# CVlab315/Domain-Adaptative-Hand-Pose-Estimation

Hardware: AMD Instinct MI355X
Metric: images/sec (unique source+target images per A+B+C training iteration, 2*B*N/t_iter) (higher is better)
Workload: dtype bf16; 1 GPU; RHD->H3D domain-adaptation iteration (steps A+B+C), resnet50 + 3-deconv neck + main head + 3 adversarial multiscale-fusion heads, 256x256, batch 64 source + 64 target per GPU, random init, synthetic batches; arch=resnet50, image_size=256, per_gpu_batch=64, global_batch=64, parallelism=dp1, hip_graphs=True, gradient_exchange=none (one rank)

## Files before the change

domain-adaptative-hand-pose-estimation_amd/csrc/api.hip:

```cpp
#include "common.h"
#include <stdarg.h>
#include <mutex>
#include <string>
#include <vector>

static thread_local char g_err[512] = "";
void mi355_set_error(const char* fmt, ...) {
  va_list ap; va_start(ap, fmt); vsnprintf(g_err, sizeof(g_err), fmt, ap); va_end(ap);
}
extern "C" const char* mi355_last_error(void) { return g_err; }
extern "C" int mi355_version(void) { return 100; }

namespace {
struct ProfState {
  std::mutex mu; bool on = false; int level = 0;
  std::vector<hipEvent_t> ev;
  std::vector<double> lflops, lbytes;
  std::vector<int> lfam; std::vector<std::string> llabel;
  size_t used = 0; double flops = 0, bytes = 0; long launches = 0;
};
ProfState& P() { static ProfState s; return s; }
thread_local char g_tag[160] = "";
}
bool prof_on() { return P().on; }
void prof_set_tag(const char* fmt, ...) {
  if (!P().on) return;
  va_list ap; va_start(ap, fmt); vsnprintf(g_tag, sizeof(g_tag), fmt, ap); va_end(ap);
}
ProfScope::ProfScope(hipStream_t st, double flops, double bytes, int family, const char* label) : s(st), on(false), slot(-1) {
  ProfState& p = P();
  if (!p.on || (family != 0 && p.level < 2)) return;
  std::lock_guard<std::mutex> lk(p.mu);
  if (p.used + 2 > p.ev.size()) {
    for (int i = 0; i < 2; ++i) { hipEvent_t e; if (hipEventCreate(&e) != hipSuccess) return; p.ev.push_back(e); }
  }
  slot = (int)p.used; p.used += 2; on = true;
  if (family == 0) { p.flops += flops; p.bytes += bytes; p.launches += 1; }
  if (p.lflops.size() < p.used / 2) { p.lflops.resize(p.used / 2); p.lbytes.resize(p.used / 2); p.lfam.resize(p.used / 2); p.llabel.resize(p.used / 2); }
  p.lflops[slot / 2] = flops; p.lbytes[slot / 2] = bytes; p.lfam[slot / 2] = family;
  p.llabel[slot / 2] = label ? label : g_tag;
  if (!label) g_tag[0] = 0;
  (void)hipEventRecord(p.ev[slot], s);
}
ProfScope::~ProfScope() {
  if (!on) return;
  ProfState& p = P();
  std::lock_guard<std::mutex> lk(p.mu);
  (void)hipEventRecord(p.ev[slot + 1], s);
}
extern "C" int mi355_prof_enable(int on) { P().on = on != 0; P().level = on; return MI355_OK; }
extern "C" int mi355_prof_reset(void) {
  ProfState& p = P(); std::lock_guard<std::mutex> lk(p.mu);
  p.used = 0; p.flops = 0; p.bytes = 0; p.launches = 0; return MI355_OK;
}
extern "C" int mi355_prof_read(double* total_ms, long* launches, double* flops, double* bytes) {
  ProfState& p = P(); std::lock_guard<std::mutex> lk(p.mu);
  double ms = 0;
  for (size_t i = 0; i + 1 < p.used; i += 2) {
    if (p.lfam[i / 2] != 0) continue;
    if (hipEventSynchronize(p.ev[i + 1]) != hipSuccess) MI_FAIL(MI355_ELAUNCH, "prof: event sync failed");
// ... 69 lines not shown
```

domain-adaptative-hand-pose-estimation_amd/csrc/common.h:

```cpp
#pragma once
#include <hip/hip_runtime.h>
#include <stdint.h>
#include <stdio.h>
#include <string.h>
#include "../../include/mi355pose.h"

typedef __bf16 bf16_t;
typedef __attribute__((ext_vector_type(8))) short bf16x8_t;
typedef __attribute__((ext_vector_type(4))) short bf16x4_t;
typedef __attribute__((ext_vector_type(16))) float f32x16_t;
typedef __attribute__((ext_vector_type(4))) float f32x4_t;

#define WAVE 64

void mi355_set_error(const char* fmt, ...);
#define MI_FAIL(code, ...) do { mi355_set_error(__VA_ARGS__); return (code); } while (0)
#define MI_CHECK_LAUNCH(name) do { hipError_t e_ = hipGetLastError(); \
  if (e_ != hipSuccess) MI_FAIL(MI355_ELAUNCH, "%s: %s", (name), hipGetErrorString(e_)); } while (0)

static inline hipStream_t as_stream(void* s) { return (hipStream_t)s; }
static inline int cdiv(long a, long b) { return (int)((a + b - 1) / b); }

template <typename T> struct Elem;
template <> struct Elem<float> {
// ... 84 lines not shown
  v = wave_max(v);
  __syncthreads();
  if ((threadIdx.x & 63) == 0) red[threadIdx.x >> 6] = v;
  __syncthreads();
  float r = red[0];
#pragma unroll
  for (int i = 1; i < NW; ++i) r = fmaxf(r, red[i]);
  return r;
}

struct FastDiv {
  unsigned mul, shr, d;
};
static inline FastDiv make_fastdiv(unsigned d) {
  FastDiv f; f.d = d;
  if (d == 1) { f.mul = 0; f.shr = 0; return f; }
  unsigned l = 0; while ((1ull << l) < d) ++l;
  unsigned long long m = ((1ull << 32) * ((1ull << l) - d)) / d + 1;
  f.mul = (unsigned)m; f.shr = l; return f;
}
__device__ inline unsigned fd_div(unsigned n, const FastDiv& f) {
  if (f.d == 1) return n;
  unsigned t = __umulhi(n, f.mul);
  return (t + ((n - t) >> 1)) >> (f.shr - 1);
}

struct ProfScope {
  hipStream_t s; bool on; int slot;
  ProfScope(hipStream_t st, double flops, double bytes = 0.0, int family = 0, const char* label = nullptr);
  ~ProfScope();
};
bool prof_on();
void prof_set_tag(const char* fmt, ...);
```

domain-adaptative-hand-pose-estimation_amd/csrc/igemm.hip:

```cpp
#include "common.h"
#include <stdlib.h>

#include "igemm_common.h"

template <typename T> struct MmaTraits;
template <> struct MmaTraits<bf16_t> { static constexpr int BK = 64; static constexpr int CH = 8; };
template <> struct MmaTraits<float> { static constexpr int BK = 32; static constexpr int CH = 4; };

#define GATHER_STAGES 1
template <typename T, int BM, int BN, int STAGES = 1, bool KW3 = false>
struct GatherSmem {
  static constexpr int kARows = KW3 ? BM + 4 * (BM / 8) + 4 : BM;
  static constexpr int kStage = (kARows + BN) * 128;
  static constexpr int kOutStride = BN * (int)sizeof(T) + 16;
  static constexpr int kOut = BM * kOutStride;
  static constexpr int kBytes = (STAGES * kStage > kOut ? STAGES * kStage : kOut) + BM * 4;
};

template <typename T, int BM, int BN, bool SMALL_C, int WGM = 2, int WGN = 2, bool HM_OUT = false, bool DMA = false, int EPI = 0,
          bool KW3 = false, bool CAT = false, int KG = 1>
__global__ __launch_bounds__(64 * WGM * WGN * KG, (KW3 && BM == 256) ? 2 : 1) void gather_gemm_kernel(const GatherArgs p) {
  constexpr int CH = MmaTraits<T>::CH;
  constexpr int GTHR = 64 * WGM * WGN;
  constexpr int NTHR = GTHR * KG, RPP = GTHR / 8;
// ... 1290 lines not shown
}

static bool t256_fits(const GatherArgs& a, long Mtot, int mode, long tmin) {
  (void)Mtot;
  long t = 0;
  for (int i = 0; i < a.nphase; ++i) t += cdiv(a.ph[i].M, 256L) * (a.Nout / 256);
  if (mode < 2) return t >= tmin && t <= 256;
  const long rem = t % 256;
  return t >= tmin && t <= 1024 && (rem == 0 || rem >= tmin);
}
template <typename T>
static int dispatch_gather(GatherArgs& a, hipStream_t st) {
  constexpr int CH = MmaTraits<T>::CH;
  if (a.Ci % CH) MI_FAIL(MI355_EINVAL, "gather: Ci=%d not a multiple of %d", a.Ci, CH);
  a.cshift = ilog2_exact(a.Ci / CH);
  if (a.cshift < 0) MI_FAIL(MI355_EINVAL, "gather: Ci/%d must be a power of two (Ci=%d)", CH, a.Ci);
  if (a.Nout % CH) MI_FAIL(MI355_EINVAL, "gather: Nout=%d not a multiple of %d", a.Nout, CH);
  if (a.nphase < 1 || a.nphase > 4) MI_FAIL(MI355_EINVAL, "gather: nphase=%d", a.nphase);
  long Mtot = 0, ntaps_tot = 0; int kchunks = 0; double flops = 0.0;
  for (int i = 0; i < a.nphase; ++i) {
    Mtot += a.ph[i].M; ntaps_tot += a.ph[i].ntaps;
    if ((a.ph[i].ntaps << a.cshift) > kchunks) kchunks = a.ph[i].ntaps << a.cshift;
    flops += 2.0 * a.ph[i].M * (double)a.Nout * a.ph[i].ntaps * a.Ci;
  }
  {
    const long imgs = a.ph[0].M / ((long)a.ph[0].OHp * a.ph[0].OWp);
    a.a_bytes = (unsigned)(imgs * a.Hi * a.Wi * a.Ci * (long)sizeof(T));
    a.b_bytes = (unsigned)((long)a.Nout * a.ldb * (long)sizeof(T));
  }
  const bool small = (a.Ci / CH) < 8;
  const long kavg = (ntaps_tot << a.cshift) / a.nphase;
  (void)kchunks;
  if (a.A2) flops += 2.0 * Mtot * (double)a.Nout * a.c2;
  ProfScope ps(st, flops, (double)a.a_bytes + (double)a.b_bytes * ntaps_tot / (a.ldb / a.Ci) + (double)Mtot * a.Nout * sizeof(T) +
                              (a.A2 ? (double)a.a2_bytes + a.b2_bytes : 0.0));
  static const int force = getenv("MI355_TILE") ? atoi(getenv("MI355_TILE")) : -1;
  static const int dma_mode = getenv("MI355_DMA") ? atoi(getenv("MI355_DMA")) : 1;
  if (a.A2) {
    if (small || a.nphase != 1 || a.out_sx != 1 || a.out_sy != 1 || a.bnb_partial || a.residual || a.accumulate)
      MI_FAIL(MI355_EINVAL, "concat-K forward: plain single-phase forward conv with >= 8 input chunks only");
    if (a.c2 < CH || a.c2 % CH || a.c2 > MmaTraits<T>::BK) MI_FAIL(MI355_EINVAL, "concat-K forward: c2=%d must be a multiple of %d and <= %d", a.c2, CH, MmaTraits<T>::BK);
    const long t128 = cdiv(Mtot, 128L) * cdiv(a.Nout, 128);
    static const int cat_tile = getenv("MI355_CAT_TILE") ? atoi(getenv("MI355_CAT_TILE")) : 0;
    static const int t256d_cat = getenv("MI355_T256D") ? atoi(getenv("MI355_T256D")) : 2;
    static const long t256d_cmin = getenv("MI355_T256D_MIN") ? atol(getenv("MI355_T256D_MIN")) : 192;
    if (t256d_cat >= 2 && sizeof(T) == 2 && a.Nout % 256 == 0 && dma_mode == 1 && t256_fits(a, Mtot, t256d_cat, t256d_cmin)) {
      if constexpr (sizeof(T) == 2) launch_gather<T, 256, 256, false, 2, 4, false, true, false, true>(a, st);
    }
    else if (cat_tile == 1 && a.Nout > 64) launch_gather<T, 128, 128, false, 2, 2, false, false, false, true>(a, st);
    else if (cat_tile == 2 && a.Nout > 64) launch_gather<T, 128, 128, false, 2, 2, false, true, false, true>(a, st);
    else if (cat_tile == 3 && a.Nout > 64) launch_gather<T, 64, 128, false, 2, 2, false, false, false, true>(a, st);
    else if (a.Nout <= 64) launch_gather<T, 64, 64, false, 2, 2, false, false, false, true>(a, st);
    else if ((dma_mode == 2) || (dma_mode == 1 && ((t128 >= 512 && kavg >= 128) || (t128 >= 256 && kavg >= 256)))) launch_gather<T, 128, 128, false, 2, 2, false, true, false, true>(a, st);
    else if (t128 >= 512 && kavg <= 32 && sizeof(T) == 2) launch_gather<T, 64, 128, false, 2, 2, false, false, false, true>(a, st);
    else if (t128 >= 512) launch_gather<T, 128, 128, false, 2, 2, false, false, false, true>(a, st);
    else if (cdiv(Mtot, 64L) * cdiv(a.Nout, 128) >= 512) launch_gather<T, 64, 128, false, 2, 2, false, false, false, true>(a, st);
    else launch_gather<T, 64, 64, false, 2, 2, false, false, false, true>(a, st);
    MI_CHECK_LAUNCH("gather_gemm_cat");
    return MI355_OK;
  }
  if constexpr (sizeof(T) == 2) {
    if (pgemm_eligible(a, 2)) return dispatch_pgemm(a, st);
  }
  if (small) { launch_gather<T, 128, 64, true>(a, st); }
  else if (force == 0) launch_gather<T, 128, 128, false>(a, st);
  else if (force == 1) launch_gather<T, 64, 128, false>(a, st);
  else if (force == 2) launch_gather<T, 128, 64, false>(a, st);
  else if (force == 3) launch_gather<T, 64, 64, false>(a, st);
  else {
    const long t128 = cdiv(Mtot, 128L) * cdiv(a.Nout, 128);
// ... 740 lines not shown
```

domain-adaptative-hand-pose-estimation_amd/csrc/igemm_common.h:

```cpp
#pragma once
#include "common.h"

#define MAX_TAPS 52
struct Tap { int8_t dy, dx; int16_t widx; };

struct Phase { int OHp, OWp, out_oy, out_ox, M, ntaps, tap0, ntm; };
struct GatherArgs {
  const void* A; const void* B; void* D;
  const float* bias; const void* residual; const float* scale;
  int Hi, Wi, Ci;
  int in_sy, in_sx;
  int Ho, Wo;
  int out_sy, out_sx;
  int Nout, ldb, ldd;
  int cshift;
  int accumulate;
  int nphase, ntn, ntiles;
  int hw;
  int lw;
  unsigned a_bytes, b_bytes;
  size_t stat_bytes;
  int stat_slices;
  const void* bnb_x; const void* bnb_y;
  const float* bnb_mean; const float* bnb_invstd; const float* bnb_gamma; const float* bnb_beta;
// ... 21 lines not shown
#pragma unroll
    for (int i = 0; i < 4; ++i)
      w[i] &= ((0u - ((mb >> (2 * i)) & 1u)) & 0x0000ffffu) | ((0u - ((mb >> (2 * i + 1)) & 1u)) & 0xffff0000u);
  } else {
#pragma unroll
    for (int i = 0; i < 4; ++i) w[i] &= 0u - ((mb >> i) & 1u);
  }
  return make_uint4(w[0], w[1], w[2], w[3]);
}

__device__ __forceinline__ int swz128(int r, int c) { return r * 128 + ((c ^ ((r >> 1) & 7)) << 4); }

__device__ __forceinline__ int xcd_remap(int bid, int nblk) {
  int q = nblk >> 3, r = nblk & 7, x = bid & 7, i = bid >> 3;
  int start = (x < r) ? x * (q + 1) : r * (q + 1) + (x - r) * q;
  return start + i;
}

typedef __attribute__((ext_vector_type(4))) unsigned int u32x4_t;
#define OOB_OFF ((int)0x80000000)
__device__ __forceinline__ __amdgpu_buffer_rsrc_t make_rsrc(const void* p, unsigned bytes) {
  return __builtin_amdgcn_make_buffer_rsrc(const_cast<void*>(p), 0, bytes, 0x00020000);
}
__device__ __forceinline__ uint4 buf_load16(__amdgpu_buffer_rsrc_t rs, int byte_off) {
  u32x4_t v = __builtin_amdgcn_raw_buffer_load_b128(rs, byte_off, 0, 0);
  return make_uint4(v[0], v[1], v[2], v[3]);
}
__device__ __forceinline__ unsigned buf_load4(__amdgpu_buffer_rsrc_t rs, int byte_off) {
  return __builtin_amdgcn_raw_buffer_load_b32(rs, byte_off, 0, 0);
}


bool pgemm_eligible(const GatherArgs& a, int elem_size);
int dispatch_pgemm(GatherArgs& a, hipStream_t st);

int dispatch_gather_fp8(GatherArgs& a, hipStream_t st);

void launch_slab_reduce(const float* ws, float* dw, long n, int S, long stride, int accumulate, hipStream_t st);
```

domain-adaptative-hand-pose-estimation_amd/csrc/pgemm.hip:

```cpp
#include "common.h"
#include <stdlib.h>

#include "igemm_common.h"

template <int BM, int BN, int NS>
struct PgSmem {
  static constexpr int kStage = BM * 128;
  static constexpr int kOut = BM * BN * 2;
  static constexpr int bytes(int nk) { return nk * BN * 128 + NS * kStage + kOut; }
};

template <int BN> __device__ __forceinline__ int out_swz(int r, int c) {
  if constexpr (BN == 128) return r * 256 + ((c ^ (r & 15)) << 4);
  else return r * 128 + ((c ^ ((r >> 1) & 7)) << 4);
}

typedef __attribute__((address_space(3))) char* lds_cptr;
__device__ __forceinline__ unsigned lds_addr(const void* p) { return (unsigned)(uintptr_t)(lds_cptr)(const_cast<void*>(p)); }
__device__ __forceinline__ bf16x8_t lds_read16(unsigned a) { bf16x8_t v; asm volatile("ds_read_b128 %0, %1" : "=v"(v) : "v"(a)); return v; }
__device__ __forceinline__ u32x4_t lds_read16u(unsigned a) { u32x4_t v; asm volatile("ds_read_b128 %0, %1" : "=v"(v) : "v"(a)); return v; }
__device__ __forceinline__ void lds_write8(unsigned a, uint2 v) { asm volatile("ds_write_b64 %0, %1" :: "v"(a), "v"(v) : "memory"); }
__device__ __forceinline__ void lds_write4(unsigned a, float v) { asm volatile("ds_write_b32 %0, %1" :: "v"(a), "v"(v) : "memory"); }
__device__ __forceinline__ float lds_read4(unsigned a) { float v; asm volatile("ds_read_b32 %0, %1" : "=v"(v) : "v"(a)); return v; }
#define LDS_WAIT_ALL() asm volatile("s_waitcnt lgkmcnt(0)" ::: "memory")
// ... 415 lines not shown
    asm volatile("s_waitcnt vmcnt(0)" ::: "memory");
    RAW_BARRIER();
    static_assert(NW * BN * 3 * 4 <= SM::kOut, "statistics scratch must fit in the staging region");
    if (lane < CPR) {
#pragma unroll
      for (int e = 0; e < CH; ++e) {
        const unsigned qa = out_base + (unsigned)(((wave * BN + ec * CH + e) * 3) * 4);
        lds_write4(qa, sn); lds_write4(qa + 4, smean[e]); lds_write4(qa + 8, sm2[e]);
      }
    }
    LDS_WAIT_ALL();
    RAW_BARRIER();
    if (t < BN && n0 + t < p.Nout) {
      float qn[NW], qm[NW], qv[NW];
#pragma unroll
      for (int w = 0; w < NW; ++w) {
        const unsigned qa = out_base + (unsigned)(((w * BN + t) * 3) * 4);
        qn[w] = lds_read4(qa); qm[w] = lds_read4(qa + 4); qv[w] = lds_read4(qa + 8);
      }
      asm volatile("s_waitcnt lgkmcnt(0)" : "+v"(qn[0]), "+v"(qn[1]), "+v"(qn[2]), "+v"(qn[3]), "+v"(qm[0]), "+v"(qm[1]), "+v"(qm[2]),
                   "+v"(qm[3]), "+v"(qv[0]), "+v"(qv[1]), "+v"(qv[2]), "+v"(qv[3]));
      float cn = 0.f, mean = 0.f, m2 = 0.f;
#pragma unroll
      for (int w = 0; w < NW; ++w) {
        const float nb = qn[w];
        if (nb > 0.f) { const float nt = cn + nb, f = nb / nt, d = qm[w] - mean; mean += d * f; m2 += qv[w] + d * d * cn * f; cn = nt; }
      }
      float* out = p.stat_partial + ((size_t)gm * p.Nout + n0 + t) * 3;
      out[0] = cn; out[1] = mean; out[2] = m2;
    }
  }
}

template <int BM, int BN, int NS, int EPI, bool ADD>
static void launch_pgemm_epi(GatherArgs& a, int ncu, int ntm, int smem, hipStream_t st) {
  auto kern = pgemm_kernel<BM, BN, NS, EPI, ADD>;
  static int attr = 0;
  if (smem > attr) { (void)hipFuncSetAttribute((const void*)kern, hipFuncAttributeMaxDynamicSharedMemorySize, smem); attr = smem; }
  static int occ_smem[4] = {0, 0, 0, 0}, occ_n[4] = {0, 0, 0, 0};
  int per_cu = 0;
  for (int i = 0; i < 4; ++i) if (occ_smem[i] == smem) per_cu = occ_n[i];
  if (!per_cu) {
    int nb = 0;
    if (hipOccupancyMaxActiveBlocksPerMultiprocessor(&nb, kern, 256, (size_t)smem) != hipSuccess || nb < 1) nb = 1;
    per_cu = nb;
    for (int i = 0; i < 4; ++i) if (!occ_smem[i]) { occ_smem[i] = smem; occ_n[i] = nb; break; }
  }
  static const int cap = getenv("MI355_PG_PER_CU") ? atoi(getenv("MI355_PG_PER_CU")) : 2;
  if (per_cu > cap) per_cu = cap;
  int groups = ncu * per_cu / a.ntn; if (groups < 1) groups = 1;
  if (groups > ntm) groups = ntm;
  if (EPI == 1) a.stat_slices = groups;
  hipLaunchKernelGGL(kern, dim3(groups * a.ntn), dim3(256), smem, st, a);
}
template <int BM, int BN, int NS>
static bool launch_pgemm(GatherArgs& a, int ncu, hipStream_t st) {
  const int nk = a.Ci >> 6;
  const bool add = a.residual || a.accumulate;
  a.pg_nadd = add ? (NS - 1) / nk + 2 : 0;
  const int smem = PgSmem<BM, BN, NS>::bytes(nk) + a.pg_nadd * (PgSmem<BM, BN, NS>::kOut + BM * BN / 8);
  if (smem > 160 * 1024) return false;
  const int ntm = cdiv(a.ph[0].M, BM);
  a.ntn = cdiv(a.Nout, BN);
  a.ph[0].ntm = ntm;
  a.ntiles = ntm * a.ntn;
  a.stat_slices = 0;
  if (a.stat_partial && (a.residual || a.accumulate || (size_t)ntm * a.Nout * 3 * sizeof(float) > a.stat_bytes)) a.stat_partial = nullptr;
  if (a.stat_partial) launch_pgemm_epi<BM, BN, NS, 1, false>(a, ncu, ntm, smem, st);
  else if (a.residual || a.accumulate) launch_pgemm_epi<BM, BN, NS, 0, true>(a, ncu, ntm, smem, st);
  else launch_pgemm_epi<BM, BN, NS, 0, false>(a, ncu, ntm, smem, st);
  return true;
}

static int g_pgemm_mode = -1;
extern "C" int mi355_set_pgemm(int mode) {
  const int prev = g_pgemm_mode;
  g_pgemm_mode = mode < 0 ? -1 : (mode > 2 ? 2 : mode);
  return prev;
}
static int pg_bn(const GatherArgs& a) {
  if (a.Nout > 64 && (long)a.Ci * 128 * 2 <= 64 * 1024) return 128;
  if ((long)a.Ci * 64 * 2 <= 64 * 1024) return 64;
  return 0;
}
bool pgemm_eligible(const GatherArgs& a, int elem_size) {
  static const int env_mode = getenv("MI355_PGEMM") ? atoi(getenv("MI355_PGEMM")) : 1;
  const int mode = g_pgemm_mode >= 0 ? g_pgemm_mode : env_mode;
  if (!mode || elem_size != 2) return false;
  if (a.nphase != 1 || a.ph[0].ntaps != 1 || a.A2) return false;
  const Tap& tp = a.taps[a.ph[0].tap0];
  if (tp.dy != 0 || tp.dx != 0 || tp.widx != 0) return false;
  if (a.in_sx != 1 || a.in_sy != 1 || a.out_sx != 1 || a.out_sy != 1) return false;
  if (a.ph[0].OHp != a.Hi || a.ph[0].OWp != a.Wi || a.Ho != a.Hi || a.Wo != a.Wi || a.ph[0].out_oy || a.ph[0].out_ox) return false;
  if (a.Ci % 64 || a.ldb != a.Ci || a.ldd != a.Nout || a.Nout % 8) return false;
  if (a.bnb_partial || a.hw) return false;
  const long Mrows = a.ph[0].M;
  if (Mrows * a.Ci * 2 >= (1L << 31) || Mrows * a.Nout * 2 >= (1L << 31)) return false;
  if (Mrows < 256 || !pg_bn(a)) return false;
  if (a.residual && a.accumulate) return false;
  if (a.acc_mask && (a.Nout % 32 || !a.accumulate)) return false;
  if (mode >= 2) return true;
  static const int add_maxk = getenv("MI355_PG_ADD") ? atoi(getenv("MI355_PG_ADD")) * 64 : 64;
  if ((a.residual || a.accumulate) && a.Ci > add_maxk) return false;
  static const long min_rows = getenv("MI355_PG_MIN_ROWS") ? atol(getenv("MI355_PG_MIN_ROWS")) : 32768;
  return Mrows >= min_rows && (a.Ci <= 128 || (a.Ci <= 256 && a.Nout <= 128));
}

int dispatch_pgemm(GatherArgs& a, hipStream_t st) {
  static int ncu = 0;
  if (!ncu) {
    int dev = 0, v = 0;
    if (hipGetDevice(&dev) != hipSuccess || hipDeviceGetAttribute(&v, hipDeviceAttributeMultiprocessorCount, dev) != hipSuccess || v < 1)
      MI_FAIL(MI355_ELAUNCH, "pgemm: cannot read the CU count");
    ncu = v;
  }
  static const int ring_env = getenv("MI355_PG_RING") ? atoi(getenv("MI355_PG_RING")) : 0;
  static const int bm = getenv("MI355_PG_BM") ? atoi(getenv("MI355_PG_BM")) : 64;
  const int bn = pg_bn(a);
  const int nk = a.Ci >> 6;
  int ring = ring_env;
  if (!ring) {
    const bool add = a.residual || a.accumulate;
    auto bytes = [&](int ns) { return nk * bn * 128 + ns * 64 * 128 + 64 * bn * 2 + (add ? ((ns - 1) / nk + 2) * (64 * bn * 2 + 64 * bn / 8) : 0); };
    if (!add) for (int ns : {8, 6, 5, 4}) if (!ring && bytes(ns) <= 80 * 1024) ring = ns;
    for (int ns : {8, 6, 5, 4}) if (!ring && bytes(ns) <= 160 * 1024) ring = ns;
    if (!ring) ring = 4;
  }
  bool ok = false;
  if (bn == 128) {
    if (bm == 128) ok = launch_pgemm<128, 128, 4>(a, ncu, st);
    else if (ring == 8) ok = launch_pgemm<64, 128, 8>(a, ncu, st);
    else if (ring == 6) ok = launch_pgemm<64, 128, 6>(a, ncu, st);
    else if (ring == 5) ok = launch_pgemm<64, 128, 5>(a, ncu, st);
    else ok = launch_pgemm<64, 128, 4>(a, ncu, st);
  } else {
    if (bm == 128) ok = launch_pgemm<128, 64, 4>(a, ncu, st);
    else if (ring == 8) ok = launch_pgemm<64, 64, 8>(a, ncu, st);
    else if (ring == 6) ok = launch_pgemm<64, 64, 6>(a, ncu, st);
    else if (ring == 5) ok = launch_pgemm<64, 64, 5>(a, ncu, st);
    else ok = launch_pgemm<64, 64, 4>(a, ncu, st);
  }
  if (!ok) MI_FAIL(MI355_EINVAL, "pgemm: the weight slice of K = %d channels does not fit LDS (bn %d)", a.Ci, bn);
  MI_CHECK_LAUNCH("pgemm");
  return MI355_OK;
}
```

profiles/insitu_table.py:

```python
import csv
import json
import re
import sys
import collections

trace, logf, iters = sys.argv[1], sys.argv[2], int(sys.argv[3])
MFMA, HBM = 1.75e15, 6.3e12

PAT = [('fwd8', 'gather_fp8_kernel'), ('dgrad8', 'gather_fp8_kernel'), ('fwd', ('gather_gemm_kernel', 'pgemm_kernel')),
       ('dgrad', ('gather_gemm_kernel', 'pgemm_kernel')), ('hm1x1', 'gather_gemm_kernel'), ('wgrad_kw_group', 'wgrad_kw_group_kernel'),
       ('wgrad_kw2', 'wgrad_kw2_kernel'), ('wgrad_kw', 'wgrad_kw_kernel'), ('wgrad_group256', 'wgrad_group256_kernel'), ('wgrad_group', 'wgrad_group_kernel'),
       ('wgrad8', 'wgrad_kw'), ('wgrad', 'wgrad_gemm_kernel'),
       ('bn_stats', 'bn_stats_kernel'), ('bn_finalize', 'bn_finalize'), ('bn_apply', 'bn_apply_kernel'), ('bn_relu_maxpool', 'bn_relu_maxpool_kernel'),
       ('bn_bwd_res', 'bn_bwd_resident_kernel'), ('bn_bwd_reduce', 'bn_bwd_reduce_kernel'), ('bn_bwd_finalize', 'bn_bwd_finalize_kernel'),
       ('bn_bwd_apply', 'bn_bwd_apply_kernel'), ('slab_reduce_group', 'slab_reduce_group_kernel'), ('slab_reduce', 'slab_reduce_kernel')]
FAMILY_KERNELS = {0: ('gather_gemm_kernel', 'gather_fp8_kernel', 'pgemm_kernel', 'wgrad_gemm_kernel', 'wgrad_kw_kernel', 'wgrad_kw2_kernel',
                      'wgrad_group_kernel', 'wgrad_group256_kernel', 'wgrad_kw_group_kernel', 'wgrad_kw8_kernel', 'wgrad_kw28_kernel'),
                  1: ('bn_stats_kernel', 'bn_finalize_kernel', 'bn_finalize_wide_kernel', 'bn_apply_kernel', 'bn_relu_maxpool_kernel',
                      'bn_bwd_resident_kernel', 'bn_bwd_reduce_kernel', 'bn_bwd_finalize_kernel', 'bn_bwd_apply_kernel'),
                  2: ('slab_reduce_kernel', 'slab_reduce_group_kernel')}


def base(name):
    m = re.match(r'_Z\d+([A-Za-z0-9_]+?)I', name)
    if m:
        return m.group(1)
    return re.sub(r'<.*|\(.*', '', re.sub(r'^void ', '', name)).strip()


log = json.load(open(logf))['launches']
rows = []
for r in csv.DictReader(open(trace)):
    rows.append((int(r['Start_Timestamp']), base(r['Kernel_Name']), r['Kernel_Name'], (int(r['End_Timestamp']) - int(r['Start_Timestamp'])) / 1e3,
                 int(r['Grid_Size_X']) // max(int(r['Workgroup_Size_X']), 1)))
rows.sort()
out = []
for fam in (0, 1, 2):
    ents = [e for e in log if e['family'] == fam]
    if not ents:
        continue
    ks = [r for r in rows if r[1] in FAMILY_KERNELS[fam]]
    if fam == 1:
        ks = [r for r in ks if not (r[1] == 'bn_bwd_reduce_kernel' and 'Lb0ELi0E' in r[2])]
    n = len(ents)
    if len(ks) < n * iters:
        print('# family %d: trace holds %d launches, fewer than %d x %d -- skipped' % (fam, len(ks), iters, n)); continue
    ks = ks[-n * iters:]
    bad = 0
    for j, e in enumerate(ents):
# ... 34 lines not shown
```

profiles/pgemm_bench.py:

```python
import os
import sys

import torch

ROOT = os.path.dirname(os.path.dirname(os.path.abspath(__file__)))
sys.path[:0] = [ROOT, os.path.join(ROOT, 'domain-adaptative-hand-pose-estimation_amd')]
import mi355
from mi355 import ops

dev = torch.device('cuda:0')
mi355.load()
dt = torch.bfloat16
LAYERS = [(64, 64, 64, 256, 8, 8), (64, 16, 256, 1024, 12, 12), (64, 32, 128, 512, 8, 8), (64, 16, 1024, 256, 10, 10),
          (64, 64, 256, 256, 3, 2), (64, 32, 512, 128, 6, 6), (64, 64, 256, 64, 4, 4), (64, 8, 512, 2048, 6, 6),
          (64, 8, 2048, 512, 4, 4), (64, 64, 256, 128, 2, 2), (64, 32, 256, 256, 3, 3), (64, 32, 512, 256, 2, 2),
          (64, 16, 1024, 512, 2, 2), (64, 64, 64, 64, 2, 2), (64, 16, 256, 256, 3, 2)]


def timeit(fn, n=20):
    for _ in range(2):
        fn()
    torch.cuda.synchronize()
    g = torch.cuda.CUDAGraph()
    st = torch.cuda.Stream()
# ... 23 lines not shown
        wf, wt = ops.pack_weights(wm, Co, 1, Ci, Ci, dt)
        x = ops.nhwc_empty(N, Ci, H, H, dt, dev).normal_()
        dy = ops.nhwc_empty(N, Co, H, H, dt, dev).normal_()
        cold = os.environ.get('COLD', '0') == '1'
        nrot = max(2, int(600e6 // (2 * N * H * H * (Ci + Co)) + 1)) if cold else 1
        xs = [x] + [x.clone() for _ in range(nrot - 1)]
        dys = [dy] + [dy.clone() for _ in range(nrot - 1)]
        rot = [0]

        def nxt(lst):
            rot[0] += 1
            return lst[rot[0] % nrot]
        M = N * H * H
        fl = 2.0 * M * Ci * Co
        by = 2.0 * (M * Ci + M * Co + Ci * Co)
        wb = wm.reshape(Co, Ci).to(dt).float()
        y = ops.conv_fwd(desc, x, wf)
        ref = x.permute(0, 2, 3, 1).reshape(M, Ci).float() @ wb.t()
        e_f = float((y.permute(0, 2, 3, 1).reshape(M, Co).float() - ref).abs().max() / (ref.abs().max() + 1e-6))
        ys, part = ops.conv_fwd_stats(desc, x, wf, None)
        e_s = float((ys.float() - y.float()).abs().max())
        dx = ops.conv_dgrad(desc, dy, wt)
        refd = dy.permute(0, 2, 3, 1).reshape(M, Co).float() @ wb
        e_d = float((dx.permute(0, 2, 3, 1).reshape(M, Ci).float() - refd).abs().max() / (refd.abs().max() + 1e-6))
        t_f = timeit(lambda: ops.conv_fwd(desc, nxt(xs), wf))
        t_s = timeit(lambda: ops.conv_fwd_stats(desc, nxt(xs), wf, None))
        t_d = timeit(lambda: ops.conv_dgrad(desc, nxt(dys), wt))
        tot['fwd'] += t_f * nf; tot['fwd_stats'] += t_s * nf; tot['dgrad'] += t_d * nd
        print('%s %4d->%4d @%2d  fwd %6.1f us %5.0f TF/s %5.0f GB/s | +stats %6.1f us | dgrad %6.1f us %5.0f TF/s | err %.1e %.1e stats-vs-plain %.1e'
              % (tag, Ci, Co, H, t_f * 1e6, fl / t_f / 1e12, by / t_f / 1e9, t_s * 1e6, t_d * 1e6, fl / t_d / 1e12, e_f, e_d, e_s), flush=True)
    print('%s per iteration: fwd %.3f ms (with statistics %.3f ms), dgrad %.3f ms' % (tag, tot['fwd'] * 1e3, tot['fwd_stats'] * 1e3, tot['dgrad'] * 1e3))


if __name__ == '__main__':
    main()
```

Baseline: 4275 images/s.

## Add full-width 256-column pointwise GEMM kernel for large 256-channel 1x1 convs

Adds a persistent pointwise GEMM kernel for 1x1 convolutions with 256 input channels and up to 256 outputs. Each 512-thread block covers the full output width, keeps all weights in registers and streams activation rows through a deep LDS ring filled by buffer-to-LDS loads. Hand-written MFMA inline asm does the math, and the epilogue can fuse bias, scale, ReLU and BN statistics, plus an optional concatenated second input. By default it is only used for large M (at least 128K rows, or 64K with concat), replacing the gather GEMM on those layers so activations are read once instead of once per column tile. The cost is a heavy register footprint and a new hand-scheduled code path that may not beat the existing kernel on every shape.

```diff
diff --git a/domain-adaptative-hand-pose-estimation_amd/csrc/api.hip b/domain-adaptative-hand-pose-estimation_amd/csrc/api.hip
--- a/domain-adaptative-hand-pose-estimation_amd/csrc/api.hip
+++ b/domain-adaptative-hand-pose-estimation_amd/csrc/api.hip
@@ -1,5 +1,6 @@
 #include "common.h"
 #include <stdarg.h>
+#include <string.h>
 #include <mutex>
 #include <string>
 #include <vector>
@@ -26,6 +27,11 @@
 void prof_set_tag(const char* fmt, ...) {
   if (!P().on) return;
   va_list ap; va_start(ap, fmt); vsnprintf(g_tag, sizeof(g_tag), fmt, ap); va_end(ap);
+}
+void prof_tag_suffix(const char* suffix) {
+  if (!P().on) return;
+  const size_t n = strlen(g_tag);
+  snprintf(g_tag + n, sizeof(g_tag) - n, "%s", suffix);
 }
 ProfScope::ProfScope(hipStream_t st, double flops, double bytes, int family, const char* label) : s(st), on(false), slot(-1) {
   ProfState& p = P();
diff --git a/domain-adaptative-hand-pose-estimation_amd/csrc/common.h b/domain-adaptative-hand-pose-estimation_amd/csrc/common.h
--- a/domain-adaptative-hand-pose-estimation_amd/csrc/common.h
+++ b/domain-adaptative-hand-pose-estimation_amd/csrc/common.h
@@ -140,3 +140,4 @@
 };
 bool prof_on();
 void prof_set_tag(const char* fmt, ...);
+void prof_tag_suffix(const char* suffix);
diff --git a/domain-adaptative-hand-pose-estimation_amd/csrc/igemm.hip b/domain-adaptative-hand-pose-estimation_amd/csrc/igemm.hip
--- a/domain-adaptative-hand-pose-estimation_amd/csrc/igemm.hip
+++ b/domain-adaptative-hand-pose-estimation_amd/csrc/igemm.hip
@@ -1346,10 +1346,13 @@
   const long kavg = (ntaps_tot << a.cshift) / a.nphase;
   (void)kchunks;
   if (a.A2) flops += 2.0 * Mtot * (double)a.Nout * a.c2;
+  const bool wide = sizeof(T) == 2 && pgemm_wide_takes(a, 2);
+  if (wide && prof_on()) prof_tag_suffix(" pgw");
   ProfScope ps(st, flops, (double)a.a_bytes + (double)a.b_bytes * ntaps_tot / (a.ldb / a.Ci) + (double)Mtot * a.Nout * sizeof(T) +
                               (a.A2 ? (double)a.a2_bytes + a.b2_bytes : 0.0));
   static const int force = getenv("MI355_TILE") ? atoi(getenv("MI355_TILE")) : -1;
   static const int dma_mode = getenv("MI355_DMA") ? atoi(getenv("MI355_DMA")) : 1;
+  if (wide) return dispatch_pgemm(a, st);
   if (a.A2) {
     if (small || a.nphase != 1 || a.out_sx != 1 || a.out_sy != 1 || a.bnb_partial || a.residual || a.accumulate)
       MI_FAIL(MI355_EINVAL, "concat-K forward: plain single-phase forward conv with >= 8 input chunks only");
diff --git a/domain-adaptative-hand-pose-estimation_amd/csrc/igemm_common.h b/domain-adaptative-hand-pose-estimation_amd/csrc/igemm_common.h
--- a/domain-adaptative-hand-pose-estimation_amd/csrc/igemm_common.h
+++ b/domain-adaptative-hand-pose-estimation_amd/csrc/igemm_common.h
@@ -77,6 +77,7 @@
 
 
 bool pgemm_eligible(const GatherArgs& a, int elem_size);
+bool pgemm_wide_takes(const GatherArgs& a, int elem_size);
 int dispatch_pgemm(GatherArgs& a, hipStream_t st);
 
 int dispatch_gather_fp8(GatherArgs& a, hipStream_t st);
diff --git a/domain-adaptative-hand-pose-estimation_amd/csrc/pgemm.hip b/domain-adaptative-hand-pose-estimation_amd/csrc/pgemm.hip
--- a/domain-adaptative-hand-pose-estimation_amd/csrc/pgemm.hip
+++ b/domain-adaptative-hand-pose-estimation_amd/csrc/pgemm.hip
@@ -471,6 +471,289 @@
   }
 }
 
+template <int NS> struct PwSmem {
+  static constexpr int kStage = 64 * 128;
+  static constexpr int kOut = 64 * 256 * 2;
+  static constexpr int bytes = NS * kStage + kOut;
+};
+__device__ __forceinline__ int out_swz256(int r, int c) { return r * 512 + ((c ^ (r & 31)) << 4); }
+
+template <bool FIRST>
+__device__ __forceinline__ void pw_step(f32x16_t& c0, f32x16_t& c1, unsigned x0, unsigned x1, unsigned x2, unsigned x3,
+                                        const bf16x8_t& b0, const bf16x8_t& b1, const bf16x8_t& b2, const bf16x8_t& b3) {
+  bf16x8_t a0, a1, e0, e1;
+#define PW_RD(DST, ADDR) "ds_read_b128 " DST ", " ADDR "\n"
+#define PW_RDH(DST, ADDR) "ds_read_b128 " DST ", " ADDR " offset:4096\n"
+#define PW_MFMA(ACC, B, A) "v_mfma_f32_32x32x16_bf16 " ACC ", " B ", " A ", " ACC "\n"
+#define PW_MFMAZ(ACC, B, A) "v_mfma_f32_32x32x16_bf16 " ACC ", " B ", " A ", 0\n"
+#define PW_BODY(M0)                                                                                                     \
+      PW_RD("%2", "%6") PW_RDH("%3", "%6") PW_RD("%4", "%7") PW_RDH("%5", "%7")                                         \
+      "s_waitcnt lgkmcnt(2)\n"                                                                                          \
+      M0                                                                                                                \
+      PW_RD("%2", "%8") PW_RDH("%3", "%8")                                                                              \
+      "s_waitcnt lgkmcnt(2)\n"                                                                                          \
+      PW_MFMA("%0", "%11", "%4") PW_MFMA("%1", "%11", "%5")                                                             \
+      PW_RD("%4", "%9") PW_RDH("%5", "%9")                                                                              \
+      "s_waitcnt lgkmcnt(2)\n"                                                                                          \
+      PW_MFMA("%0", "%12", "%2") PW_MFMA("%1", "%12", "%3")                                                             \
+      "s_waitcnt lgkmcnt(0)\n"                                                                                          \
+      PW_MFMA("%0", "%13", "%4") PW_MFMA("%1", "%13", "%5")
+  if constexpr (FIRST) {
+    asm volatile(PW_BODY(PW_MFMAZ("%0", "%10", "%2") PW_MFMAZ("%1", "%10", "%3"))
+                 : "+v"(c0), "+v"(c1), "=&v"(a0), "=&v"(a1), "=&v"(e0), "=&v"(e1)
+                 : "v"(x0), "v"(x1), "v"(x2), "v"(x3), "v"(b0), "v"(b1), "v"(b2), "v"(b3) : "memory");
+  } else {
+    asm volatile(PW_BODY(PW_MFMA("%0", "%10", "%2") PW_MFMA("%1", "%10", "%3"))
+                 : "+v"(c0), "+v"(c1), "=&v"(a0), "=&v"(a1), "=&v"(e0), "=&v"(e1)
+                 : "v"(x0), "v"(x1), "v"(x2), "v"(x3), "v"(b0), "v"(b1), "v"(b2), "v"(b3) : "memory");
+  }
+#undef PW_BODY
+#undef PW_MFMAZ
+#undef PW_MFMA
+#undef PW_RDH
+#undef PW_RD
+}
+
+template <int NK, bool CAT, int NS, int EPI>
+__global__ __launch_bounds__(512) void pgemm_wide_kernel(const GatherArgs p) {
+  constexpr int CH = 8, NTHR = 512, BM = 64, BN = 256;
+  constexpr int NKT = NK + (CAT ? 1 : 0);
+  constexpr int DIST = NS - 1;
+  constexpr int CPR = BN / CH;
+  constexpr int IT = BM * CPR / NTHR;
+  constexpr int RSTEP = NTHR / CPR;
+  using SM = PwSmem<NS>;
+  extern __shared__ __attribute__((aligned(16))) char smem[];
+
+  const int t = threadIdx.x, lane = t & 63, wave = t >> 6;
+  const int wave_u = __builtin_amdgcn_readfirstlane(wave);
+  const int wn0 = wave * 32;
+  const unsigned smem_base = lds_addr(smem);
+  const int lc = t & 7, lr = t >> 3;
+  const int lcs = lc ^ ((lr >> 1) & 7);
+  const int r31 = lane & 31, hi = lane >> 5;
+  const int M = p.ph[0].M, K = NK * 64, ntm = p.ph[0].ntm;
+  const int G = (int)gridDim.x, gm = (int)blockIdx.x;
+  const int my_tiles = gm < ntm ? (ntm - gm + G - 1) / G : 0;
+  const int total = my_tiles * NKT;
+  if (total == 0) return;
+  const unsigned ring_base = smem_base, out_base = ring_base + (unsigned)(NS * SM::kStage);
+
+  const __amdgpu_buffer_rsrc_t rsA = make_rsrc(p.A, p.a_bytes), rsB = make_rsrc(p.B, p.b_bytes);
+  const __amdgpu_buffer_rsrc_t rsA2 = make_rsrc(CAT ? p.A2 : p.A, CAT ? p.a2_bytes : 0u), rsB2 = make_rsrc(CAT ? p.B2 : p.B, CAT ? p.b2_bytes : 0u);
+  (void)rsA; (void)rsB; (void)rsA2; (void)rsB2; (void)wave_u;
+
+  int is_tile = 0, is_kt = 0, is_gs = 0, is_slot = 0;
+  int voffA = OOB_OFF, voffA2 = OOB_OFF;
+  auto set_issue_tile = [&](int i) {
+    const int m = (gm + i * G) * BM + lr;
+    voffA = m < M ? (m * K + lcs * CH) * 2 : OOB_OFF;
+    if constexpr (CAT) voffA2 = (m < M && lcs * CH < p.c2) ? (m * p.c2 + lcs * CH) * 2 : OOB_OFF;
+  };
+  auto issue = [&]() {
+#if defined(__HIP_DEVICE_COMPILE__)
+    typedef __attribute__((address_space(3))) void* ldsp;
+    char* sa = smem + is_slot * SM::kStage + wave_u * 1024;
+    if (CAT && is_kt == NK) __builtin_amdgcn_raw_ptr_buffer_load_lds(rsA2, (ldsp)sa, 16, voffA2, 0, 0, 0);
+    else __builtin_amdgcn_raw_ptr_buffer_load_lds(rsA, (ldsp)sa, 16, voffA, is_kt * 128, 0, 0);
+#endif
+    ++is_gs;
+    if (++is_slot == NS) is_slot = 0;
+    if (++is_kt == NKT) { is_kt = 0; ++is_tile; if (is_tile < my_tiles) set_issue_tile(is_tile); }
+  };
+  set_issue_tile(0);
+#pragma unroll
+  for (int d = 0; d < DIST; ++d)
+    if (is_gs < total) issue();
+
+  bf16x8_t bw[NKT][4];
+  {
+    const int n = wn0 + r31;
+#pragma unroll
+    for (int kt = 0; kt < NK; ++kt)
+#pragma unroll
+      for (int s = 0; s < 4; ++s) {
+        u32x4_t v = {0u, 0u, 0u, 0u};
+#if defined(__HIP_DEVICE_COMPILE__)
+        v = __builtin_amdgcn_raw_buffer_load_b128(rsB, n < p.Nout ? (n * p.ldb + kt * 64 + (2 * s + hi) * CH) * 2 : OOB_OFF, 0, 0);
+#endif
+        bw[kt][s] = __builtin_bit_cast(bf16x8_t, v);
+      }
+    if constexpr (CAT) {
+#pragma unroll
+      for (int s = 0; s < 4; ++s) {
+        u32x4_t v = {0u, 0u, 0u, 0u};
+#if defined(__HIP_DEVICE_COMPILE__)
+        v = __builtin_amdgcn_raw_buffer_load_b128(rsB2, (n < p.Nout && (2 * s + hi) * CH < p.c2) ? (n * p.c2 + (2 * s + hi) * CH) * 2 : OOB_OFF, 0, 0);
+#endif
+        bw[NK][s] = __builtin_bit_cast(bf16x8_t, v);
+      }
+    }
+  }
+  float4 bq[4];
+#pragma unroll
+  for (int g = 0; g < 4; ++g) {
+    const int n = wn0 + 8 * g + 4 * hi;
+    bq[g] = (p.bias && n < p.Nout) ? *reinterpret_cast<const float4*>(p.bias + n) : make_float4(0.f, 0.f, 0.f, 0.f);
+    if constexpr (CAT) if (p.bias2 && n < p.Nout) {
+      const float4 b2 = *reinterpret_cast<const float4*>(p.bias2 + n);
+      bq[g].x += b2.x; bq[g].y += b2.y; bq[g].z += b2.z; bq[g].w += b2.w;
+    }
+  }
+  const float scale = p.scale ? *p.scale : 1.0f;
+  const bool affine = p.bias != nullptr || p.scale != nullptr || (CAT && p.bias2 != nullptr);
+#pragma unroll
+  for (int kt = 0; kt < NKT; ++kt)
+#pragma unroll
+    for (int s = 0; s < 4; ++s) asm volatile("" : "+v"(bw[kt][s]));
+#pragma unroll
+  for (int g = 0; g < 4; ++g) asm volatile("" : "+v"(bq[g].x), "+v"(bq[g].y), "+v"(bq[g].z), "+v"(bq[g].w));
+
+  f32x16_t acc0, acc1;
+#pragma unroll
+  for (int r = 0; r < 16; ++r) { acc0[r] = 0.f; acc1[r] = 0.f; }
+  unsigned fa[4];
+#pragma unroll
+  for (int s = 0; s < 4; ++s) fa[s] = (unsigned)swz128(r31, 2 * s + hi);
+
+  unsigned so[4];
+#pragma unroll
+  for (int g = 0; g < 4; ++g) { const int nl = wn0 + 8 * g + 4 * hi; so[g] = (unsigned)(out_swz256(r31, nl >> 3) + (nl & 7) * 2); }
+  bf16_t* __restrict__ D = reinterpret_cast<bf16_t*>(p.D);
+  const bool plain = !p.relu;
+  const int ec = t % CPR, er0 = t / CPR;
+  unsigned rd[IT];
+#pragma unroll
+  for (int k = 0; k < IT; ++k) rd[k] = (unsigned)out_swz256(er0 + k * RSTEP, ec);
+  constexpr bool stats = EPI == 1;
+  float st_n = 0.f, st_ref[CH], st_s[CH], st_q[CH];
+#pragma unroll
+  for (int e = 0; e < CH; ++e) { st_ref[e] = 0.f; st_s[e] = 0.f; st_q[e] = 0.f; }
+  auto epilogue = [&](int tm) {
+    const int m0 = tm * BM;
+    const int n = ec * CH;
+    const int rows_left = M - (m0 + er0);
+    const size_t g0 = (size_t)(m0 + er0) * p.ldd + n;
+    asm volatile("s_nop 7\n\ts_nop 7" ::: "memory");
+#pragma unroll
+    for (int i = 0; i < 2; ++i)
+#pragma unroll
+      for (int g = 0; g < 4; ++g) {
+        const float bb[4] = {bq[g].x, bq[g].y, bq[g].z, bq[g].w};
+        union { bf16_t h[4]; uint2 q; } u;
+#pragma unroll
+        for (int e = 0; e < 4; ++e) {
+          const float a = i ? acc1[4 * g + e] : acc0[4 * g + e];
+          u.h[e] = affine ? (bf16_t)((a + bb[e]) * scale) : (bf16_t)a;
+        }
+        lds_write8(out_base + so[g] + (unsigned)(i * 32 * BN * 2), u.q);
+      }
+    LDS_WAIT_ALL();
+    RAW_BARRIER();
+    u32x4_t q[IT];
+#pragma unroll
+    for (int k = 0; k < IT; ++k) q[k] = lds_read16u(out_base + rd[k]);
+#pragma unroll
+    for (int k = 0; k < IT; ++k) {
+      asm volatile("s_waitcnt lgkmcnt(%1)" : "+v"(q[k]) : "n"(IT - 1 - k));
+      if (k * RSTEP >= rows_left || n >= p.Nout) continue;
+      const size_t g = g0 + (size_t)k * RSTEP * p.ldd;
+      const uint4 qk = make_uint4(q[k][0], q[k][1], q[k][2], q[k][3]);
+      if (!stats && plain) { *reinterpret_cast<uint4*>(D + g) = qk; continue; }
+      float v[CH]; Chunk<bf16_t>::unpack(qk, v);
+      if (stats) {
+        if (st_n == 0.f) {
+#pragma unroll
+          for (int e = 0; e < CH; ++e) st_ref[e] = v[e];
+        }
+        st_n += 1.f;
+#pragma unroll
+        for (int e = 0; e < CH; ++e) { const float d = v[e] - st_ref[e]; st_s[e] += d; st_q[e] += d * d; }
+        if (plain) { *reinterpret_cast<uint4*>(D + g) = qk; continue; }
+      }
+#pragma unroll
+      for (int e = 0; e < CH; ++e) v[e] = v[e] < 0.f ? 0.f : v[e];
+      Chunk<bf16_t>::store(D + g, v);
+    }
+  };
+
+  int gs = 0;
+  unsigned epi_hist = 0;
+  int cur_slot = 0;
+  for (int tile_i = 0; tile_i < my_tiles; ++tile_i) {
+#pragma unroll
+    for (int kt = 0; kt < NKT; ++kt, ++gs) {
+      if (DIST > 1 && gs + DIST - 1 < total) {
+        const int c = __builtin_popcount(epi_hist & ((1u << DIST) - 1u));
+        wait_vm_dyn(__builtin_amdgcn_readfirstlane((DIST - 1) + c * IT));
+      } else {
+        asm volatile("s_waitcnt vmcnt(0)" ::: "memory");
+      }
+      RAW_BARRIER();
+      if (is_gs < total) issue();
+      const unsigned as = ring_base + (unsigned)(cur_slot * SM::kStage);
+      if (++cur_slot == NS) cur_slot = 0;
+      __builtin_amdgcn_s_setprio(1);
+      if (kt == 0) pw_step<true>(acc0, acc1, as + fa[0], as + fa[1], as + fa[2], as + fa[3], bw[kt][0], bw[kt][1], bw[kt][2], bw[kt][3]);
+      else pw_step<false>(acc0, acc1, as + fa[0], as + fa[1], as + fa[2], as + fa[3], bw[kt][0], bw[kt][1], bw[kt][2], bw[kt][3]);
+      __builtin_amdgcn_s_setprio(0);
+      epi_hist <<= 1;
+    }
+    const int tm = gm + tile_i * G;
+    epilogue(tm);
+    if ((tm + 1) * BM <= M && p.Nout == BN) epi_hist |= 1u;
+  }
+  if constexpr (stats) {
+    constexpr int NW = NTHR / 64;
+    float sn = st_n, smean[CH], sm2[CH];
+    const float inv = sn > 0.f ? 1.f / sn : 0.f;
+#pragma unroll
+    for (int e = 0; e < CH; ++e) { smean[e] = st_ref[e] + st_s[e] * inv; sm2[e] = st_q[e] - st_s[e] * st_s[e] * inv; sm2[e] = sm2[e] < 0.f ? 0.f : sm2[e]; }
+#pragma unroll
+    for (int o = CPR; o < 64; o <<= 1) {
+      const float nb = __shfl_down(sn, o, 64);
+      const float nt = sn + nb, f = nt > 0.f ? nb / nt : 0.f;
+#pragma unroll
+      for (int e = 0; e < CH; ++e) {
+        const float mb = __shfl_down(smean[e], o, 64), vb = __shfl_down(sm2[e], o, 64);
+        const float d = mb - smean[e];
+        smean[e] += d * f; sm2[e] += vb + d * d * sn * f;
+      }
+      sn = nt;
+    }
+    asm volatile("s_waitcnt vmcnt(0)" ::: "memory");
+    RAW_BARRIER();
+    static_assert(NW * BN * 3 * 4 <= SM::kOut, "statistics scratch must fit in the staging region");
+    if (lane < CPR) {
+#pragma unroll
+      for (int e = 0; e < CH; ++e) {
+        const unsigned qa = out_base + (unsigned)(((wave * BN + ec * CH + e) * 3) * 4);
+        lds_write4(qa, sn); lds_write4(qa + 4, smean[e]); lds_write4(qa + 8, sm2[e]);
+      }
+    }
+    LDS_WAIT_ALL();
+    RAW_BARRIER();
+    if (t < BN && t < p.Nout) {
+      float qn[NW], qm[NW], qv[NW];
+#pragma unroll
+      for (int w = 0; w < NW; ++w) {
+        const unsigned qa = out_base + (unsigned)(((w * BN + t) * 3) * 4);
+        qn[w] = lds_read4(qa); qm[w] = lds_read4(qa + 4); qv[w] = lds_read4(qa + 8);
+      }
+#pragma unroll
+      for (int w = 0; w < NW; ++w) asm volatile("s_waitcnt lgkmcnt(0)" : "+v"(qn[w]), "+v"(qm[w]), "+v"(qv[w]));
+      float cn = 0.f, mean = 0.f, m2 = 0.f;
+#pragma unroll
+      for (int w = 0; w < NW; ++w) {
+        const float nb = qn[w];
+        if (nb > 0.f) { const float nt = cn + nb, f = nb / nt, d = qm[w] - mean; mean += d * f; m2 += qv[w] + d * d * cn * f; cn = nt; }
+      }
+      float* out = p.stat_partial + ((size_t)gm * p.Nout + t) * 3;
+      out[0] = cn; out[1] = mean; out[2] = m2;
+    }
+  }
+}
+
 template <int BM, int BN, int NS, int EPI, bool ADD>
 static void launch_pgemm_epi(GatherArgs& a, int ncu, int ntm, int smem, hipStream_t st) {
   auto kern = pgemm_kernel<BM, BN, NS, EPI, ADD>;
@@ -511,22 +794,52 @@
   return true;
 }
 
+template <int NK, bool CAT, int NS, int EPI>
+static void launch_pgemm_wide_epi(GatherArgs& a, int ncu, int ntm, hipStream_t st) {
+  auto kern = pgemm_wide_kernel<NK, CAT, NS, EPI>;
+  constexpr int smem = PwSmem<NS>::bytes;
+  static int per_cu = 0;
+  if (!per_cu) {
+    (void)hipFuncSetAttribute((const void*)kern, hipFuncAttributeMaxDynamicSharedMemorySize, smem);
+    int nb = 0;
+    if (hipOccupancyMaxActiveBlocksPerMultiprocessor(&nb, kern, 512, (size_t)smem) != hipSuccess || nb < 1) nb = 1;
+    per_cu = nb;
+  }
+  int groups = ncu * per_cu; if (groups > ntm) groups = ntm;
+  if (EPI == 1) a.stat_slices = groups;
+  hipLaunchKernelGGL(kern, dim3(groups), dim3(512), smem, st, a);
+}
+static void launch_pgemm_wide(GatherArgs& a, int ncu, hipStream_t st) {
+  constexpr int NS = 8, NS_CAT = 12;
+  const int ntm = cdiv(a.ph[0].M, 64);
+  a.ntn = 1; a.ph[0].ntm = ntm; a.ntiles = ntm; a.stat_slices = 0; a.pg_nadd = 0;
+  if (a.stat_partial && (size_t)ntm * a.Nout * 3 * sizeof(float) > a.stat_bytes) a.stat_partial = nullptr;
+  if (a.A2) {
+    if (a.stat_partial) launch_pgemm_wide_epi<4, true, NS_CAT, 1>(a, ncu, ntm, st);
+    else launch_pgemm_wide_epi<4, true, NS_CAT, 0>(a, ncu, ntm, st);
+  } else {
+    if (a.stat_partial) launch_pgemm_wide_epi<4, false, NS, 1>(a, ncu, ntm, st);
+    else launch_pgemm_wide_epi<4, false, NS, 0>(a, ncu, ntm, st);
+  }
+}
+
 static int g_pgemm_mode = -1;
 extern "C" int mi355_set_pgemm(int mode) {
   const int prev = g_pgemm_mode;
   g_pgemm_mode = mode < 0 ? -1 : (mode > 2 ? 2 : mode);
   return prev;
 }
+static int pg_mode() {
+  static const int env_mode = getenv("MI355_PGEMM") ? atoi(getenv("MI355_PGEMM")) : 1;
+  return g_pgemm_mode >= 0 ? g_pgemm_mode : env_mode;
+}
 static int pg_bn(const GatherArgs& a) {
   if (a.Nout > 64 && (long)a.Ci * 128 * 2 <= 64 * 1024) return 128;
   if ((long)a.Ci * 64 * 2 <= 64 * 1024) return 64;
   return 0;
 }
-bool pgemm_eligible(const GatherArgs& a, int elem_size) {
-  static const int env_mode = getenv("MI355_PGEMM") ? atoi(getenv("MI355_PGEMM")) : 1;
-  const int mode = g_pgemm_mode >= 0 ? g_pgemm_mode : env_mode;
-  if (!mode || elem_size != 2) return false;
-  if (a.nphase != 1 || a.ph[0].ntaps != 1 || a.A2) return false;
+static bool pg_shape_ok(const GatherArgs& a) {
+  if (a.nphase != 1 || a.ph[0].ntaps != 1) return false;
   const Tap& tp = a.taps[a.ph[0].tap0];
   if (tp.dy != 0 || tp.dx != 0 || tp.widx != 0) return false;
   if (a.in_sx != 1 || a.in_sy != 1 || a.out_sx != 1 || a.out_sy != 1) return false;
@@ -535,7 +848,28 @@
   if (a.bnb_partial || a.hw) return false;
   const long Mrows = a.ph[0].M;
   if (Mrows * a.Ci * 2 >= (1L << 31) || Mrows * a.Nout * 2 >= (1L << 31)) return false;
-  if (Mrows < 256 || !pg_bn(a)) return false;
+  return Mrows >= 256;
+}
+static bool pg_wide_fits(const GatherArgs& a) {
+  if (!pg_shape_ok(a)) return false;
+  if (a.Ci != 256 || a.Nout <= 128 || a.Nout > 256) return false;
+  if (a.residual || a.accumulate || a.acc_mask) return false;
+  if (a.A2 && (!a.B2 || a.c2 < 8 || a.c2 > 64 || a.c2 % 8 || (long)a.ph[0].M * a.c2 * 2 >= (1L << 31))) return false;
+  return true;
+}
+bool pgemm_wide_takes(const GatherArgs& a, int elem_size) {
+  const int mode = pg_mode();
+  if (!mode || elem_size != 2 || !pg_wide_fits(a)) return false;
+  if (mode >= 2) return true;
+  return a.ph[0].M >= (a.A2 ? 65536 : 131072);
+}
+bool pgemm_eligible(const GatherArgs& a, int elem_size) {
+  const int mode = pg_mode();
+  if (!mode || elem_size != 2) return false;
+  if (pgemm_wide_takes(a, elem_size)) return true;
+  if (a.A2 || !pg_shape_ok(a)) return false;
+  const long Mrows = a.ph[0].M;
+  if (!pg_bn(a)) return false;
   if (a.residual && a.accumulate) return false;
   if (a.acc_mask && (a.Nout % 32 || !a.accumulate)) return false;
   if (mode >= 2) return true;
@@ -552,6 +886,11 @@
     if (hipGetDevice(&dev) != hipSuccess || hipDeviceGetAttribute(&v, hipDeviceAttributeMultiprocessorCount, dev) != hipSuccess || v < 1)
       MI_FAIL(MI355_ELAUNCH, "pgemm: cannot read the CU count");
     ncu = v;
+  }
+  if (pgemm_wide_takes(a, 2)) {
+    launch_pgemm_wide(a, ncu, st);
+    MI_CHECK_LAUNCH("pgemm_wide");
+    return MI355_OK;
   }
   static const int ring_env = getenv("MI355_PG_RING") ? atoi(getenv("MI355_PG_RING")) : 0;
   static const int bm = getenv("MI355_PG_BM") ? atoi(getenv("MI355_PG_BM")) : 64;
diff --git a/profiles/insitu_table.py b/profiles/insitu_table.py
--- a/profiles/insitu_table.py
+++ b/profiles/insitu_table.py
@@ -7,14 +7,14 @@
 trace, logf, iters = sys.argv[1], sys.argv[2], int(sys.argv[3])
 MFMA, HBM = 1.75e15, 6.3e12
 
-PAT = [('fwd8', 'gather_fp8_kernel'), ('dgrad8', 'gather_fp8_kernel'), ('fwd', ('gather_gemm_kernel', 'pgemm_kernel')),
-       ('dgrad', ('gather_gemm_kernel', 'pgemm_kernel')), ('hm1x1', 'gather_gemm_kernel'), ('wgrad_kw_group', 'wgrad_kw_group_kernel'),
+PAT = [('fwd8', 'gather_fp8_kernel'), ('dgrad8', 'gather_fp8_kernel'), ('fwd', ('gather_gemm_kernel', 'pgemm_kernel', 'pgemm_wide_kernel')),
+       ('dgrad', ('gather_gemm_kernel', 'pgemm_kernel', 'pgemm_wide_kernel')), ('hm1x1', 'gather_gemm_kernel'), ('wgrad_kw_group', 'wgrad_kw_group_kernel'),
        ('wgrad_kw2', 'wgrad_kw2_kernel'), ('wgrad_kw', 'wgrad_kw_kernel'), ('wgrad_group256', 'wgrad_group256_kernel'), ('wgrad_group', 'wgrad_group_kernel'),
        ('wgrad8', 'wgrad_kw'), ('wgrad', 'wgrad_gemm_kernel'),
        ('bn_stats', 'bn_stats_kernel'), ('bn_finalize', 'bn_finalize'), ('bn_apply', 'bn_apply_kernel'), ('bn_relu_maxpool', 'bn_relu_maxpool_kernel'),
        ('bn_bwd_res', 'bn_bwd_resident_kernel'), ('bn_bwd_reduce', 'bn_bwd_reduce_kernel'), ('bn_bwd_finalize', 'bn_bwd_finalize_kernel'),
        ('bn_bwd_apply', 'bn_bwd_apply_kernel'), ('slab_reduce_group', 'slab_reduce_group_kernel'), ('slab_reduce', 'slab_reduce_kernel')]
-FAMILY_KERNELS = {0: ('gather_gemm_kernel', 'gather_fp8_kernel', 'pgemm_kernel', 'wgrad_gemm_kernel', 'wgrad_kw_kernel', 'wgrad_kw2_kernel',
+FAMILY_KERNELS = {0: ('gather_gemm_kernel', 'gather_fp8_kernel', 'pgemm_kernel', 'pgemm_wide_kernel', 'wgrad_gemm_kernel', 'wgrad_kw_kernel', 'wgrad_kw2_kernel',
                       'wgrad_group_kernel', 'wgrad_group256_kernel', 'wgrad_kw_group_kernel', 'wgrad_kw8_kernel', 'wgrad_kw28_kernel'),
                   1: ('bn_stats_kernel', 'bn_finalize_kernel', 'bn_finalize_wide_kernel', 'bn_apply_kernel', 'bn_relu_maxpool_kernel',
                       'bn_bwd_resident_kernel', 'bn_bwd_reduce_kernel', 'bn_bwd_finalize_kernel', 'bn_bwd_apply_kernel'),
diff --git a/profiles/pgemm_bench.py b/profiles/pgemm_bench.py
--- a/profiles/pgemm_bench.py
+++ b/profiles/pgemm_bench.py
@@ -79,5 +79,51 @@
     print('%s per iteration: fwd %.3f ms (with statistics %.3f ms), dgrad %.3f ms' % (tag, tot['fwd'] * 1e3, tot['fwd_stats'] * 1e3, tot['dgrad'] * 1e3))
 
 
+def wide():
+    lib = mi355.load()
+    g = torch.Generator(device='cpu').manual_seed(5)
+    for N, H in ((64, 64), (64, 32)):
+        Ci = Co = 256
+        desc = ops.make_desc(N, H, H, Ci, Co, 1, 1, 1, 0, dt)
+        wm = (torch.randn(Co, 1, 1, Ci, generator=g) * 0.05).to(dev)
+        wf, wt = ops.pack_weights(wm, Co, 1, Ci, Ci, dt)
+        w2 = (torch.randn(Co, 32, generator=g) * 0.2).to(dev).to(dt)
+        b1, b2 = torch.randn(Co, generator=g).to(dev), torch.randn(Co, generator=g).to(dev)
+        M = N * H * H
+        nrot = max(2, int(600e6 // (2 * M * (Ci + Co)) + 1))
+        xs = [ops.nhwc_empty(N, Ci, H, H, dt, dev).normal_() for _ in range(nrot)]
+        hs = [ops.nhwc_empty(N, 32, H, H, dt, dev).normal_() for _ in range(nrot)]
+        outs = [ops.nhwc_empty(N, Ci, H, H, dt, dev).normal_() for _ in range(nrot)]
+        rot = [0]
+
+        def nxt(lst):
+            rot[0] += 1
+            return lst[rot[0] % nrot]
+        forms = [('fwd +stats +cat', lambda: ops.conv_fwd_cat(desc, nxt(xs), wf, b1, hs[rot[0] % nrot], w2, b2, want_stats=True), 2.0 * M * (Ci + 32 + Co)),
+                 ('fwd +stats', lambda: ops.conv_fwd_stats(desc, nxt(xs), wf, None), 2.0 * M * (Ci + Co)),
+                 ('dgrad', lambda: ops.conv_dgrad(desc, nxt(xs), wt), 2.0 * M * (Ci + Co)),
+                 ('dgrad +acc', lambda: ops.conv_dgrad(desc, nxt(xs), wt, out=outs[rot[0] % nrot], accumulate=True), 2.0 * M * (Ci + 2 * Co))]
+        for name, fn, by in forms:
+            row = []
+            for mode in (0, 2):
+                prev = lib.mi355_set_pgemm(mode)
+                try:
+                    ops.prof_enable(1); ops.prof_reset()
+                    fn(); torch.cuda.synchronize()
+                    lab = [e['label'] for e in ops.prof_launches() if e['family'] == 0][-1]
+                    ops.prof_reset(); ops.prof_enable(0)
+                    ts = sorted(timeit(fn) for _ in range(3))
+                finally:
+                    lib.mi355_set_pgemm(prev)
+                row.append((lab, ts))
+            (l0, t0), (l2, t2) = row
+            print('%-16s 256>256 @%dx%d  gather %6.1f us (%5.1f .. %5.1f) %5.0f GB/s | mode 2 %6.1f us (%5.1f .. %5.1f) %5.0f GB/s  [%s]'
+                  % (name, H, H, t0[1] * 1e6, t0[0] * 1e6, t0[2] * 1e6, by / t0[1] / 1e9, t2[1] * 1e6, t2[0] * 1e6, t2[2] * 1e6, by / t2[1] / 1e9,
+                     'full-width build' if l2.endswith(' pgw') else 'not taken: ' + l2), flush=True)
+
+
 if __name__ == '__main__':
-    main()
+    if len(sys.argv) > 1 and sys.argv[1] == 'wide':
+        wide()
+    else:
+        main()
```

Result: no change. 4312 images/s (median of 6 runs) (+0.9%).
